# lilijiangg/AutoDiffusion

Hardware: AMD Instinct MI355X
Metric: images/sec (node), ADM-G ImageNet-64 4-step DDIM (higher is better)
Workload: dtype bf16

## Files before the change

autodiffusion_amd/csrc/adm_conv1x1.hip:

```cpp
#include <stdlib.h>

#include <type_traits>

#include "adm_common.h"
#include "adm_conv_internal.h"

namespace {

typedef __attribute__((ext_vector_type(4))) unsigned int u32x4;
typedef float f32x2 __attribute__((ext_vector_type(2)));
constexpr unsigned OOB = 0x80000000u;

struct Conv1K {
  const uint16_t* in0; const uint16_t* in1; const uint16_t* w; const uint16_t* res;
  const float* bias; const float* aa; const float* ab; uint16_t* out; float* stats;
  int N, HW, C0, C1, Cout, ntiles16, stat_slabs, m_tiles, nblocks_n;
  int csplit, nbper;
  unsigned wbytes, rcp_seg;
};

__device__ __forceinline__ uint4 bufload16(__amdgpu_buffer_rsrc_t r, unsigned voff, unsigned soff) {
  const u32x4 v = __builtin_amdgcn_raw_buffer_load_b128(r, (int)voff, (int)soff, 0);
  return make_uint4(v[0], v[1], v[2], v[3]);
}

template <int BM>
constexpr int c1_stg_bytes() {
  constexpr int a = BM * (192 * 2 + 16), b = (512 / 24) * 192 * 8, c = 8 * 4096;
  return a > b ? (a > c ? a : c) : (b > c ? b : c);
}
template <int BM>
constexpr int c1_lds_bytes(int k) { return BM * (2 * k + 32) + c1_stg_bytes<BM>() + 2 * k * 4; }

template <int BM, int PRO, bool WP, int WM, bool GG = false>
__global__ void __launch_bounds__(512, 2)
conv1x1r_kernel(const Conv1K p) {
  constexpr int NT = 512, WN = 8 / WM, BN = WN * 48, TM = BM / 16 / WM, TN = 3, BNH = 192;
  constexpr int EROW = BNH * 2 + 16, SEGS = BNH / 8, PR = NT / SEGS, NIT = (BM + PR - 1) / PR;
  constexpr int WROW = 112, WST = 4096;
  extern __shared__ __attribute__((aligned(16))) unsigned char smem[];
  const int K = p.C0 + p.C1, RB = 2 * K + 32, ksteps = K / 32, segk = K / 8;
  unsigned char* const A = smem;
  unsigned char* const stg = smem + BM * RB;
  float* const tab = reinterpret_cast<float*>(stg + c1_stg_bytes<BM>());

  const int tid = threadIdx.x, lane = tid & 63;
  const int wave = __builtin_amdgcn_readfirstlane(tid >> 6);
  const int lc = lane & 15, lq = lane >> 4;
  const int wm = wave / WN, wn = wave % WN;
  const __amdgpu_buffer_rsrc_t rsw = __builtin_amdgcn_make_buffer_rsrc((void*)p.w, 0, p.wbytes, 0x00020000);
  const __amdgpu_buffer_rsrc_t rsb = __builtin_amdgcn_make_buffer_rsrc((void*)p.bias, 0, p.Cout * 4, 0x00020000);
  const unsigned wstep = (unsigned)p.ntiles16 * 1024u;

  const int xcd = blockIdx.x & 7;
  const int gx = (int)(gridDim.x >> 3) + (xcd < (int)(gridDim.x & 7));
  const int tcount = (p.m_tiles >> 3) + (xcd < (p.m_tiles & 7));
  const int tstart = xcd * (p.m_tiles >> 3) + min(xcd, p.m_tiles & 7);

  for (int tl = blockIdx.x >> 3; tl < tcount; tl += gx) {
    const int tq = tstart + tl;
    const int pt = p.csplit > 1 ? tq / p.csplit : tq;
    const int nb0 = p.csplit > 1 ? (tq - pt * p.csplit) * p.nbper : 0;
    const int nb1 = p.csplit > 1 ? min(p.nblocks_n, nb0 + p.nbper) : p.nblocks_n;
    const int pb = pt * BM;
    const int img = pb / p.HW;
    __syncthreads();
    if constexpr (PRO != 0) {
      for (int i = tid; i < 2 * K / 4; i += NT) {
        const int half = i >= K / 4, j = half ? i - K / 4 : i;
        *reinterpret_cast<float4*>(tab + half * K + j * 4) =
            *reinterpret_cast<const float4*>((half ? p.ab : p.aa) + (long long)img * K + j * 4);
      }
      __syncthreads();
    }
    for (int i0 = 0; i0 < BM * segk; i0 += 4 * NT) {
      uint4 v[4];
      int px[4], sg[4];
#pragma unroll
      for (int u = 0; u < 4; ++u) {
        const int idx = i0 + u * NT + tid;
        px[u] = (int)__umulhi((unsigned)idx, p.rcp_seg);
        sg[u] = idx - px[u] * segk;
        v[u] = make_uint4(0, 0, 0, 0);
        if (px[u] < BM) {
          const int ch = sg[u] * 8;
          const long long pix = (long long)pb + px[u];
          v[u] = ch < p.C0 ? *reinterpret_cast<const uint4*>(p.in0 + pix * p.C0 + ch)
                           : *reinterpret_cast<const uint4*>(p.in1 + pix * p.C1 + (ch - p.C0));
        }
      }
#pragma unroll
      for (int u = 0; u < 4; ++u) {
        if (px[u] >= BM) continue;
        uint4 o = v[u];
        if constexpr (PRO != 0) {
          const float* ta = tab + sg[u] * 8;
          float a8[8], b8[8];
          *reinterpret_cast<float4*>(a8) = *reinterpret_cast<const float4*>(ta);
          *reinterpret_cast<float4*>(a8 + 4) = *reinterpret_cast<const float4*>(ta + 4);
          *reinterpret_cast<float4*>(b8) = *reinterpret_cast<const float4*>(ta + K);
          *reinterpret_cast<float4*>(b8 + 4) = *reinterpret_cast<const float4*>(ta + K + 4);
          uint32_t w4[4] = {o.x, o.y, o.z, o.w};
#pragma unroll
          for (int j = 0; j < 4; ++j) {
            float lo = adm_lo_f32(w4[j]), hi = adm_hi_f32(w4[j]);
            lo = a8[2 * j] * lo + b8[2 * j];
            hi = a8[2 * j + 1] * hi + b8[2 * j + 1];
            if constexpr (PRO == 2) { lo = adm_silu(lo); hi = adm_silu(hi); }
            w4[j] = adm_pack2(lo, hi);
          }
          o = make_uint4(w4[0], w4[1], w4[2], w4[3]);
        }
        *reinterpret_cast<uint4*>(A + px[u] * RB + sg[u] * 16) = o;
      }
    }
    __syncthreads();

    const unsigned char* const alane = A + (wm * TM * 16 + lc) * RB + lq * 16;
    for (int nb = nb0; nb < nb1; ++nb) {
      unsigned wofs[TN];
      f32x4 acc[TM][TN];
#pragma unroll
      for (int j = 0; j < TN; ++j) {
        const int t16 = nb * (BN / 16) + wn * TN + j;
        wofs[j] = t16 < p.ntiles16 ? (unsigned)((t16 * 64 + lane) * 16) : OOB;
        const int bch = t16 * 16 + lq * 4;
        const uint4 b = bufload16(rsb, bch + 3 < p.Cout ? (unsigned)bch * 4u : OOB, 0);
#pragma unroll
        for (int i = 0; i < TM; ++i)
          acc[i][j] = f32x4{__uint_as_float(b.x), __uint_as_float(b.y), __uint_as_float(b.z), __uint_as_float(b.w)};
      }
      auto load_w = [&](int step, uint4 (&dst)[TN]) {
#pragma unroll
        for (int j = 0; j < TN; ++j) dst[j] = bufload16(rsw, wofs[j], (unsigned)step * wstep);
      };
      auto kstep = [&](int ks, const uint4 (&w)[TN]) {
        constexpr int AFD = TM < 4 ? TM : 4;
        const unsigned char* ak = alane + ks * 64;
        __builtin_amdgcn_sched_barrier(0);
        adm_h8 af[TM];
#pragma unroll
        for (int i = 0; i < AFD; ++i) af[i] = *reinterpret_cast<const adm_h8*>(ak + i * 16 * RB);
#pragma unroll
        for (int i = 0; i < TM; ++i) {
          if (i + AFD < TM) af[i + AFD] = *reinterpret_cast<const adm_h8*>(ak + (i + AFD) * 16 * RB);
#pragma unroll
          for (int j = 0; j < TN; ++j)
            acc[i][j] = adm_mfma_16x16x32(__builtin_bit_cast(adm_h8, w[j]), af[i], acc[i][j], 0, 0, 0);
        }
#pragma unroll
        for (int i = 0; i < AFD; ++i) __builtin_amdgcn_sched_group_barrier(0x100, 1, 0);
#pragma unroll
        for (int i = 0; i < TM; ++i) {
          if (i + AFD < TM) __builtin_amdgcn_sched_group_barrier(0x100, 1, 0);
          __builtin_amdgcn_sched_group_barrier(0x008, TN, 0);
        }
      };
      uint4 wr[4][TN];
      const int last = ksteps - 1;
      load_w(0, wr[0]);
      load_w(min(1, last), wr[1]);
      load_w(min(2, last), wr[2]);
      int k0 = 0;
      for (; k0 + 3 <= last; k0 += 4) {
        load_w(min(k0 + 3, last), wr[3]); kstep(k0, wr[0]);
        load_w(min(k0 + 4, last), wr[0]); kstep(k0 + 1, wr[1]);
        load_w(min(k0 + 5, last), wr[1]); kstep(k0 + 2, wr[2]);
        load_w(min(k0 + 6, last), wr[2]); kstep(k0 + 3, wr[3]);
      }
      if (k0 <= last) kstep(k0, wr[0]);
      if (k0 + 1 <= last) kstep(k0 + 1, wr[1]);
      if (k0 + 2 <= last) kstep(k0 + 2, wr[2]);

      if constexpr (GG) {
      const int cbw = nb * BN + wn * 48;
      if (cbw < p.Cout) {
        unsigned char* const wst = stg + wave * WST;
        const int Co = p.Cout >> 1, cbo = cbw >> 1;
        const int sgl = lane % 3, rowl = lane / 3;
        const bool lact = lane < 63 && cbo + sgl * 8 < Co;
#pragma unroll
        for (int c = 0; c < TM / 2; ++c) {
#pragma unroll
          for (int ii = 0; ii < 2; ++ii)
#pragma unroll
            for (int j = 0; j < TN; ++j) {
              const f32x4 v = acc[2 * c + ii][j];
              const float y0 = v[0] * (0.5f * v[1] * (1.0f + erff(v[1] * 0.70710678118654752f)));
              const float y1 = v[2] * (0.5f * v[3] * (1.0f + erff(v[3] * 0.70710678118654752f)));
              *reinterpret_cast<uint32_t*>(wst + (ii * 16 + lc) * 64 + (j * 8 + lq * 2) * 2) = adm_pack2(y0, y1);
            }
#pragma unroll
          for (int q = 0; q < 2; ++q) {
            const int r = rowl + q * 21;
            if (!lact || r >= 32) continue;
            const long long eo = ((long long)pb + c * 32 + r) * Co + cbo + sgl * 8;
            *reinterpret_cast<uint4*>(p.out + eo) = *reinterpret_cast<const uint4*>(wst + r * 64 + sgl * 16);
          }
        }
      }
      } else if constexpr (WP) {
      const int cbw = nb * BN + wn * 48;
      if (cbw < p.Cout) {
        unsigned char* const wst = stg + wave * WST;
        const int sgl = lane % 6, rowl = lane / 6;
        const bool lact = lane < 60 && cbw + sgl * 8 < p.Cout;
        f32x2 s1[4], s2[4];
#pragma unroll
        for (int q = 0; q < 4; ++q) { s1[q] = f32x2{0.f, 0.f}; s2[q] = f32x2{0.f, 0.f}; }
#pragma unroll
        for (int c = 0; c < TM / 2; ++c) {
#pragma unroll
          for (int ii = 0; ii < 2; ++ii)
#pragma unroll
            for (int j = 0; j < TN; ++j) {
              const f32x4 v = acc[2 * c + ii][j];
              uint2 o;
              o.x = adm_pack2(v[0], v[1]);
              o.y = adm_pack2(v[2], v[3]);
              *reinterpret_cast<uint2*>(wst + (ii * 16 + lc) * WROW + (j * 16 + lq * 4) * 2) = o;
            }
#pragma unroll
          for (int q = 0; q < 4; ++q) {
            const int r = rowl + q * 10;
            if (!lact || r >= 32) continue;
            const long long eo = ((long long)pb + wm * TM * 16 + c * 32 + r) * p.Cout + cbw + sgl * 8;
            uint4 v = *reinterpret_cast<const uint4*>(wst + r * WROW + sgl * 16);
            uint32_t a4[4] = {v.x, v.y, v.z, v.w};
            if (p.res) {
              const uint4 rr = *reinterpret_cast<const uint4*>(p.res + eo);
              const uint32_t r4[4] = {rr.x, rr.y, rr.z, rr.w};
#pragma unroll
              for (int e = 0; e < 4; ++e) {
                const f32x2 t = f32x2{adm_lo_f32(a4[e]), adm_hi_f32(a4[e])} +
                                f32x2{adm_lo_f32(r4[e]), adm_hi_f32(r4[e])};
                a4[e] = adm_pack2(t.x, t.y);
              }
              v = make_uint4(a4[0], a4[1], a4[2], a4[3]);
            }
            *reinterpret_cast<uint4*>(p.out + eo) = v;
#pragma unroll
            for (int e = 0; e < 4; ++e) {
              const f32x2 t = f32x2{adm_lo_f32(a4[e]), adm_hi_f32(a4[e])};
              s1[e] += t;
              s2[e] = __builtin_elementwise_fma(t, t, s2[e]);
            }
          }
        }
        if (p.stats) {
          float* red = reinterpret_cast<float*>(wst);
          if (lane < 60) {
#pragma unroll
            for (int e = 0; e < 8; ++e) {
              red[(rowl * 48 + sgl * 8 + e) * 2 + 0] = s1[e >> 1][e & 1];
              red[(rowl * 48 + sgl * 8 + e) * 2 + 1] = s2[e >> 1][e & 1];
            }
          }
          if (lane < 48 && cbw + lane < p.Cout) {
            float t1 = 0.f, t2 = 0.f;
#pragma unroll
            for (int q = 0; q < 10; ++q) { t1 += red[(q * 48 + lane) * 2]; t2 += red[(q * 48 + lane) * 2 + 1]; }
            const int slab = ((pb - img * p.HW) / BM) * WM + wm;
            float* dst = p.stats + (((long long)img * p.stat_slabs + slab) * p.Cout + cbw + lane) * 2;
            dst[0] = t1;
            dst[1] = t2;
          }
        }
      }
      } else {
      const int sgo = tid % SEGS, prow = tid / SEGS;
#pragma unroll 1
      for (int hf = 0; hf < BN / BNH; ++hf) {
        const int cb = nb * BN + hf * BNH;
        if (cb >= p.Cout) break;
        __syncthreads();
        if (WM == 2 || (wave >> 2) == hf) {
#pragma unroll
          for (int j = 0; j < TN; ++j) {
            const int ch0 = ((wn & 3) * TN + j) * 16 + lq * 4;
#pragma unroll
            for (int i = 0; i < TM; ++i) {
              uint2 o;
              o.x = adm_pack2(acc[i][j][0], acc[i][j][1]);
              o.y = adm_pack2(acc[i][j][2], acc[i][j][3]);
              *reinterpret_cast<uint2*>(stg + ((wm * TM + i) * 16 + lc) * EROW + ch0 * 2) = o;
            }
          }
        }
        const int gch = cb + sgo * 8;
        const bool act = prow < PR && gch < p.Cout;
        uint4 rr[NIT];
#pragma unroll
        for (int k = 0; k < NIT; ++k) {
          const int m = prow + k * PR;
          rr[k] = make_uint4(0, 0, 0, 0);
          if (p.res && act && m < BM) rr[k] = *reinterpret_cast<const uint4*>(p.res + ((long long)pb + m) * p.Cout + gch);
        }
        __syncthreads();
        f32x2 s1[4], s2[4];
#pragma unroll
        for (int q = 0; q < 4; ++q) { s1[q] = f32x2{0.f, 0.f}; s2[q] = f32x2{0.f, 0.f}; }
#pragma unroll
        for (int k = 0; k < NIT; ++k) {
          const int m = prow + k * PR;
          if (!act || m >= BM) continue;
          uint4 v = *reinterpret_cast<const uint4*>(stg + m * EROW + sgo * 16);
          uint32_t a4[4] = {v.x, v.y, v.z, v.w};
          if (p.res) {
            const uint32_t r4[4] = {rr[k].x, rr[k].y, rr[k].z, rr[k].w};
#pragma unroll
            for (int q = 0; q < 4; ++q) {
              const f32x2 t = f32x2{adm_lo_f32(a4[q]), adm_hi_f32(a4[q])} +
                              f32x2{adm_lo_f32(r4[q]), adm_hi_f32(r4[q])};
              a4[q] = adm_pack2(t.x, t.y);
            }
            v = make_uint4(a4[0], a4[1], a4[2], a4[3]);
          }
          *reinterpret_cast<uint4*>(p.out + ((long long)pb + m) * p.Cout + gch) = v;
#pragma unroll
          for (int q = 0; q < 4; ++q) {
            const f32x2 t = f32x2{adm_lo_f32(a4[q]), adm_hi_f32(a4[q])};
            s1[q] += t;
            s2[q] = __builtin_elementwise_fma(t, t, s2[q]);
          }
        }
        if (p.stats) {
          float* red = reinterpret_cast<float*>(stg);
          __syncthreads();
          if (prow < PR) {
#pragma unroll
            for (int e = 0; e < 8; ++e) {
              red[(prow * BNH + sgo * 8 + e) * 2 + 0] = s1[e >> 1][e & 1];
              red[(prow * BNH + sgo * 8 + e) * 2 + 1] = s2[e >> 1][e & 1];
            }
          }
          __syncthreads();
          if (tid < BNH && cb + tid < p.Cout) {
            float t1 = 0.f, t2 = 0.f;
            for (int q = 0; q < PR; ++q) { t1 += red[(q * BNH + tid) * 2]; t2 += red[(q * BNH + tid) * 2 + 1]; }
            const int slab = ((pb - img * p.HW) / BM) * WM;
            float* dst = p.stats + (((long long)img * p.stat_slabs + slab) * p.Cout + cb + tid) * 2;
            dst[0] = t1;
            dst[1] = t2;
            if (WM == 2) { dst[2 * p.Cout] = 0.f; dst[2 * p.Cout + 1] = 0.f; }
          }
        }
      }
      }
    }
  }
}

template <int BM, int PRO, bool WP, int WM, bool GG = false>
int launch_c1(const Conv1K& k, int smem, hipStream_t s) {
  static int slots_dev[64] = {};
  int dev = 0;
  (void)hipGetDevice(&dev);
  int& slots = slots_dev[dev & 63];
  const void* fn = reinterpret_cast<const void*>(&conv1x1r_kernel<BM, PRO, WP, WM, GG>);
  if (slots == 0) {
    hipError_t e = hipFuncSetAttribute(fn, hipFuncAttributeMaxDynamicSharedMemorySize, 160 * 1024);
    if (e != hipSuccess) ADM_FAIL((int)e, "adm_conv (1x1 resident): hipFuncSetAttribute: %s", hipGetErrorString(e));
    int ncu = 0;
    e = hipDeviceGetAttribute(&ncu, hipDeviceAttributeMultiprocessorCount, dev);
    if (e != hipSuccess || ncu <= 0) ADM_FAIL((int)e, "adm_conv: hipDeviceGetAttribute: %s", hipGetErrorString(e));
    slots = ncu;
  }
  const int mine = adm_stream_cus((void*)s, slots);
  const unsigned blocks = (unsigned)(k.m_tiles < mine ? k.m_tiles : mine);
  hipLaunchKernelGGL((conv1x1r_kernel<BM, PRO, WP, WM, GG>), dim3(blocks), dim3(512), smem, s, k);
  return adm_check_launch("adm_conv");
}

}

int adm_conv1x1_resident_cfg(const adm_conv_args* a, int* wm_out) {
  static const bool disabled = getenv("ADM_CONV_NO_RESIDENT") != nullptr;
  if (disabled && a->variant == 0 && !a->geglu) return 0;
  if (a->taps != 1 || a->out_mode != 0 || (a->variant != 0 && a->variant != 10) || a->ksplit > 1) return 0;
  const int k = a->c0 + a->c1, hw = a->h * a->w;
  if (k % 64 != 0 || a->c0 % 8 != 0 || a->c1 % 8 != 0 || a->cout % 8 != 0 || hw % 64 != 0) return 0;
  if (a->variant == 0 && a->cout < 256) return 0;
  if (a->geglu && (a->res || a->out_stats || a->prologue != 0 || a->cout % 16 != 0 || a->cout <= 192)) return 0;
  if (wm_out) *wm_out = a->cout <= 192 ? 2 : 1;
  const int lim = 160 * 1024;
  if (hw % 128 == 0 && c1_lds_bytes<128>(k) <= lim) return 128;
  if (c1_lds_bytes<64>(k) <= lim) return 64;
  static const bool bm32 = getenv("ADM_C1_BM32") != nullptr;
  if (k >= 1280 && hw <= 256 && hw % 32 == 0 && a->cout > 192 && (a->variant == 10 || (bm32 && a->cout <= 1536)) && c1_lds_bytes<32>(k) <= lim) return 32;
  return 0;
}

int adm_conv1x1_resident_slabs(const adm_conv_args* a) {
  int wm = 1;
  const int bm = adm_conv1x1_resident_cfg(a, &wm);
  return bm ? a->h * a->w / bm * wm : 0;
}

template <int BM, int WM>
static int launch_c1_cfg(const adm_conv_args* a, const Conv1K& k, int smem, hipStream_t s) {
  const bool wp = a->res == nullptr;
  switch (a->prologue) {
    case 0: return wp ? launch_c1<BM, 0, true, WM>(k, smem, s) : launch_c1<BM, 0, false, WM>(k, smem, s);
    case 1: return wp ? launch_c1<BM, 1, true, WM>(k, smem, s) : launch_c1<BM, 1, false, WM>(k, smem, s);
    default: return wp ? launch_c1<BM, 2, true, WM>(k, smem, s) : launch_c1<BM, 2, false, WM>(k, smem, s);
  }
}

int adm_conv1x1_resident_launch(const adm_conv_args* a, void* stream) {
  int wm = 1;
  const int bm = adm_conv1x1_resident_cfg(a, &wm);
  Conv1K k{};
  k.in0 = a->in0; k.in1 = a->in1; k.w = a->w_packed; k.res = a->res;
  k.bias = a->bias; k.aa = a->aff_a; k.ab = a->aff_b; k.out = (uint16_t*)a->out; k.stats = a->out_stats;
  k.N = a->n; k.HW = a->h * a->w; k.C0 = a->c0; k.C1 = a->c1; k.Cout = a->cout;
  k.ntiles16 = (a->cout + 15) / 16;
  k.stat_slabs = k.HW / bm * wm;
  k.m_tiles = (int)((long long)a->n * k.HW / bm);
  const int bn = wm == 1 ? 384 : 192;
  k.nblocks_n = (a->cout + bn - 1) / bn;
  k.csplit = 1;
  {
    static const bool no_csplit = getenv("ADM_C1_NO_CSPLIT") != nullptr;
    static int ncu_dev[64] = {};
    int dev = 0;
    (void)hipGetDevice(&dev);
    int& ncu_c = ncu_dev[dev & 63];
    if (ncu_c == 0 && (hipDeviceGetAttribute(&ncu_c, hipDeviceAttributeMultiprocessorCount, dev) != hipSuccess || ncu_c <= 0)) ncu_c = 256;
    const int ncu = ncu_c;
    if (!no_csplit && k.nblocks_n > 1 && k.m_tiles < ncu) {
      int want = (ncu + k.m_tiles - 1) / k.m_tiles;
      if (want > k.nblocks_n) want = k.nblocks_n;
      if (want > 4) want = 4;
      k.csplit = want;
    }
  }
  k.nbper = (k.nblocks_n + k.csplit - 1) / k.csplit;
  k.csplit = (k.nblocks_n + k.nbper - 1) / k.nbper;
  k.m_tiles *= k.csplit;
  const int kk = a->c0 + a->c1;
  k.wbytes = (unsigned)(((long long)kk / 32) * k.ntiles16 * 1024);
  const unsigned segk = (unsigned)kk / 8;
  k.rcp_seg = (unsigned)(((1ull << 32) + segk - 1) / segk);
  hipStream_t s = (hipStream_t)stream;
  const int smem = bm == 128 ? c1_lds_bytes<128>(kk) : (bm == 64 ? c1_lds_bytes<64>(kk) : c1_lds_bytes<32>(kk));
  if (a->geglu)
    return bm == 128 ? launch_c1<128, 0, true, 1, true>(k, smem, s)
                     : (bm == 64 ? launch_c1<64, 0, true, 1, true>(k, smem, s) : launch_c1<32, 0, true, 1, true>(k, smem, s));
  if (bm == 128) return wm == 1 ? launch_c1_cfg<128, 1>(a, k, smem, s) : launch_c1_cfg<128, 2>(a, k, smem, s);
  if (bm == 32) return launch_c1_cfg<32, 1>(a, k, smem, s);
  return wm == 1 ? launch_c1_cfg<64, 1>(a, k, smem, s) : launch_c1_cfg<64, 2>(a, k, smem, s);
}
```

Measured before the change: 803.8.

## Pipeline activation staging into LDS chunk-by-chunk with the K-loop MFMAs

Instead of loading and transforming the whole activation tile into LDS before any MFMA work, the 1x1 conv kernel now stages the first 128-channel chunk up front. It then fetches and parks each following chunk while the previous chunks' k-steps run, during the first output-column block. The goal is to hide global-load latency of the prologue behind matrix work. This adds a block-wide barrier per chunk and extra registers for the in-flight chunk, which may reduce occupancy. It is enabled by default when K > 128 and divisible by 64, and can be disabled with an environment variable.

```diff
diff --git a/autodiffusion_amd/csrc/adm_conv1x1.hip b/autodiffusion_amd/csrc/adm_conv1x1.hip
--- a/autodiffusion_amd/csrc/adm_conv1x1.hip
+++ b/autodiffusion_amd/csrc/adm_conv1x1.hip
@@ -16,8 +16,11 @@
   const float* bias; const float* aa; const float* ab; uint16_t* out; float* stats;
   int N, HW, C0, C1, Cout, ntiles16, stat_slabs, m_tiles, nblocks_n;
   int csplit, nbper;
+  int kpipe;
   unsigned wbytes, rcp_seg;
 };
+
+constexpr int C1_KC = 128;
 
 __device__ __forceinline__ uint4 bufload16(__amdgpu_buffer_rsrc_t r, unsigned voff, unsigned soff) {
   const u32x4 v = __builtin_amdgcn_raw_buffer_load_b128(r, (int)voff, (int)soff, 0);
@@ -73,45 +76,72 @@
       }
       __syncthreads();
     }
-    for (int i0 = 0; i0 < BM * segk; i0 += 4 * NT) {
-      uint4 v[4];
-      int px[4], sg[4];
-#pragma unroll
-      for (int u = 0; u < 4; ++u) {
-        const int idx = i0 + u * NT + tid;
-        px[u] = (int)__umulhi((unsigned)idx, p.rcp_seg);
-        sg[u] = idx - px[u] * segk;
+    int ft = tid;
+    asm volatile("" : "+v"(ft));
+    auto park = [&](int px, int sg, uint4 o) {
+      if constexpr (PRO != 0) {
+        const float* ta = tab + sg * 8;
+        float a8[8], b8[8];
+        *reinterpret_cast<float4*>(a8) = *reinterpret_cast<const float4*>(ta);
+        *reinterpret_cast<float4*>(a8 + 4) = *reinterpret_cast<const float4*>(ta + 4);
+        *reinterpret_cast<float4*>(b8) = *reinterpret_cast<const float4*>(ta + K);
+        *reinterpret_cast<float4*>(b8 + 4) = *reinterpret_cast<const float4*>(ta + K + 4);
+        uint32_t w4[4] = {o.x, o.y, o.z, o.w};
+#pragma unroll
+        for (int j = 0; j < 4; ++j) {
+          float lo = adm_lo_f32(w4[j]), hi = adm_hi_f32(w4[j]);
+          lo = a8[2 * j] * lo + b8[2 * j];
+          hi = a8[2 * j + 1] * hi + b8[2 * j + 1];
+          if constexpr (PRO == 2) { lo = adm_silu(lo); hi = adm_silu(hi); }
+          w4[j] = adm_pack2(lo, hi);
+        }
+        o = make_uint4(w4[0], w4[1], w4[2], w4[3]);
+      }
+      *reinterpret_cast<uint4*>(A + px * RB + sg * 16) = o;
+    };
+    auto fetch = [&](int px, int sg) {
+      const int ch = sg * 8;
+      const long long pix = (long long)pb + px;
+      return ch < p.C0 ? *reinterpret_cast<const uint4*>(p.in0 + pix * p.C0 + ch)
+                       : *reinterpret_cast<const uint4*>(p.in1 + pix * p.C1 + (ch - p.C0));
+    };
+    constexpr int CV = BM * (C1_KC / 8) / NT;
+    auto chunk_load = [&](int c, uint4 (&v)[CV]) {
+      const int sh = K - c * C1_KC >= C1_KC ? 4 : 3;
+#pragma unroll
+      for (int u = 0; u < CV; ++u) {
+        const int idx = u * NT + ft, px = idx >> sh;
         v[u] = make_uint4(0, 0, 0, 0);
-        if (px[u] < BM) {
-          const int ch = sg[u] * 8;
-          const long long pix = (long long)pb + px[u];
-          v[u] = ch < p.C0 ? *reinterpret_cast<const uint4*>(p.in0 + pix * p.C0 + ch)
-                           : *reinterpret_cast<const uint4*>(p.in1 + pix * p.C1 + (ch - p.C0));
-        }
-      }
-#pragma unroll
-      for (int u = 0; u < 4; ++u) {
-        if (px[u] >= BM) continue;
-        uint4 o = v[u];
-        if constexpr (PRO != 0) {
-          const float* ta = tab + sg[u] * 8;
-          float a8[8], b8[8];
-          *reinterpret_cast<float4*>(a8) = *reinterpret_cast<const float4*>(ta);
-          *reinterpret_cast<float4*>(a8 + 4) = *reinterpret_cast<const float4*>(ta + 4);
-          *reinterpret_cast<float4*>(b8) = *reinterpret_cast<const float4*>(ta + K);
-          *reinterpret_cast<float4*>(b8 + 4) = *reinterpret_cast<const float4*>(ta + K + 4);
-          uint32_t w4[4] = {o.x, o.y, o.z, o.w};
-#pragma unroll
-          for (int j = 0; j < 4; ++j) {
-            float lo = adm_lo_f32(w4[j]), hi = adm_hi_f32(w4[j]);
-            lo = a8[2 * j] * lo + b8[2 * j];
-            hi = a8[2 * j + 1] * hi + b8[2 * j + 1];
-            if constexpr (PRO == 2) { lo = adm_silu(lo); hi = adm_silu(hi); }
-            w4[j] = adm_pack2(lo, hi);
-          }
-          o = make_uint4(w4[0], w4[1], w4[2], w4[3]);
-        }
-        *reinterpret_cast<uint4*>(A + px[u] * RB + sg[u] * 16) = o;
+        if (px < BM) v[u] = fetch(px, c * (C1_KC / 8) + (idx & ((1 << sh) - 1)));
+      }
+    };
+    auto chunk_park = [&](int c, const uint4 (&v)[CV]) {
+      const int sh = K - c * C1_KC >= C1_KC ? 4 : 3;
+#pragma unroll
+      for (int u = 0; u < CV; ++u) {
+        const int idx = u * NT + ft, px = idx >> sh;
+        if (px < BM) park(px, c * (C1_KC / 8) + (idx & ((1 << sh) - 1)), v[u]);
+      }
+    };
+    if (p.kpipe) {
+      uint4 v[CV];
+      chunk_load(0, v);
+      chunk_park(0, v);
+    } else {
+      for (int i0 = 0; i0 < BM * segk; i0 += 4 * NT) {
+        uint4 v[4];
+        int px[4], sg[4];
+#pragma unroll
+        for (int u = 0; u < 4; ++u) {
+          const int idx = i0 + u * NT + ft;
+          px[u] = (int)__umulhi((unsigned)idx, p.rcp_seg);
+          sg[u] = idx - px[u] * segk;
+          v[u] = make_uint4(0, 0, 0, 0);
+          if (px[u] < BM) v[u] = fetch(px[u], sg[u]);
+        }
+#pragma unroll
+        for (int u = 0; u < 4; ++u)
+          if (px[u] < BM) park(px[u], sg[u], v[u]);
       }
     }
     __syncthreads();
@@ -156,21 +186,32 @@
           __builtin_amdgcn_sched_group_barrier(0x008, TN, 0);
         }
       };
-      uint4 wr[4][TN];
-      const int last = ksteps - 1;
-      load_w(0, wr[0]);
-      load_w(min(1, last), wr[1]);
-      load_w(min(2, last), wr[2]);
-      int k0 = 0;
-      for (; k0 + 3 <= last; k0 += 4) {
-        load_w(min(k0 + 3, last), wr[3]); kstep(k0, wr[0]);
-        load_w(min(k0 + 4, last), wr[0]); kstep(k0 + 1, wr[1]);
-        load_w(min(k0 + 5, last), wr[1]); kstep(k0 + 2, wr[2]);
-        load_w(min(k0 + 6, last), wr[2]); kstep(k0 + 3, wr[3]);
-      }
-      if (k0 <= last) kstep(k0, wr[0]);
-      if (k0 + 1 <= last) kstep(k0 + 1, wr[1]);
-      if (k0 + 2 <= last) kstep(k0 + 2, wr[2]);
+      {
+        const bool pipe = p.kpipe && nb == nb0;
+        uint4 wr[4][TN];
+        uint4 cv[CV];
+        const int last = ksteps - 1;
+        load_w(0, wr[0]);
+        load_w(min(1, last), wr[1]);
+        load_w(min(2, last), wr[2]);
+        int k0 = 0;
+        for (; k0 + 3 <= last; k0 += 4) {
+          load_w(min(k0 + 3, last), wr[3]);
+          const bool more = pipe && k0 + 4 <= last;
+          if (more) chunk_load((k0 >> 2) + 1, cv);
+          kstep(k0, wr[0]);
+          load_w(min(k0 + 4, last), wr[0]); kstep(k0 + 1, wr[1]);
+          load_w(min(k0 + 5, last), wr[1]); kstep(k0 + 2, wr[2]);
+          load_w(min(k0 + 6, last), wr[2]); kstep(k0 + 3, wr[3]);
+          if (more) {
+            chunk_park((k0 >> 2) + 1, cv);
+            __syncthreads();
+          }
+        }
+        if (k0 <= last) kstep(k0, wr[0]);
+        if (k0 + 1 <= last) kstep(k0 + 1, wr[1]);
+        if (k0 + 2 <= last) kstep(k0 + 2, wr[2]);
+      }
 
       if constexpr (GG) {
       const int cbw = nb * BN + wn * 48;
@@ -439,6 +480,10 @@
   k.csplit = (k.nblocks_n + k.nbper - 1) / k.nbper;
   k.m_tiles *= k.csplit;
   const int kk = a->c0 + a->c1;
+  {
+    static const bool no_kpipe = getenv("ADM_C1_NO_KPIPE") != nullptr;
+    k.kpipe = !no_kpipe && kk > C1_KC && kk % 64 == 0;
+  }
   k.wbytes = (unsigned)(((long long)kk / 32) * k.ntiles16 * 1024);
   const unsigned segk = (unsigned)kk / 8;
   k.rcp_seg = (unsigned)(((1ull << 32) + segk - 1) / segk);
```

Result: no change. 802.5 (-0.2%).
